# nurturenature/jepsen-tigerbeetle

Measured on AMD Instinct MI355X. Metric: histories/sec, 10k-op/64-proc cas-register histories (time-to-verdict ms in extra), higher is better.
Workload: dtype u64

## Files before the change

### jepsen-tigerbeetle_amd/csrc/batch_run.hip

```cpp
#include "tbc_batch.h"
#include "witness_expand.h"

using namespace tbc;

namespace tbc {

static SearchArgs make_search_args(tbc_batch* B, uint64_t* tab, uint32_t n_work) {
  SearchArgs a{};
  a.hist = B->d_hist.p; a.rec = B->d_rec.p; a.seg = B->d_seg.p; a.ret_slot = B->d_ret_slot.p;
  a.ret_op = B->d_ret_op.p;
  a.frames = B->d_frames.p; a.tab = tab; a.results = B->d_results.p;
  a.witness = B->opts.want_witness ? B->d_witness.p : nullptr;
  a.work = B->d_work.p; a.queue = B->d_queue.p;
  a.table = B->d_table.p; a.n_work = n_work; a.model_kind = B->model.kind;
  a.init_state = B->model.init;
  a.n_classes = B->model.n_classes; a.n_states = B->model.n_states;
  a.max_steps = B->opts.max_steps;
  a.time_limit_ticks = B->opts.time_limit_ms * 100000ull;
  a.dbg = debug_words();
  a.pool_vals = B->d_pool_vals.p;
  a.cfg = B->d_cfg.p;
  a.progress = B->progress; a.progress_dev = B->d_progress.p;
  return a;
}
// ... 352 lines not shown
        restart_budget((ph == 0 && !b->sweep && b->order_restarts_apply()) ? 32ull * b->max_ops : 0ull),
        stall_on(b->lanes != 0 && (b->opts.dominance & TBC_DOM_STALL_HANDOVER) != 0 && !b->count_form && b->mask_words == 1 && !b->opts.want_witness && b->opts.max_steps == 0 && ph == 0 &&
                 (b->model.kind == TBC_MODEL_REGISTER || b->model.kind == TBC_MODEL_CAS_REGISTER) && b->vpad != 0),
        was_handed(b->n_hist, 0), rs_level(b->n_hist, kInf), rs_valid(b->n_hist, 0),
        max_bytes(b->opts.max_visited_bytes ? b->opts.max_visited_bytes : (1ull << 30)) {
    if (B->sweep || B->rsweep) {
      swa.hist = B->d_hist.p; swa.bh = B->d_bh.p; swa.off = B->d_off.p; swa.ncr = B->d_ncr.p; swa.lst = B->d_lst.p;
      swa.crashed = B->d_crashed.p; swa.twn = B->reg_rules() ? B->d_twn.p : nullptr; swa.rdm = B->reg_rules() ? B->d_rdm.p : nullptr;
      swa.slot8 = B->d_slot8.p; swa.cuts = B->d_cuts.p; swa.seg = B->d_sres.p; swa.table = B->d_table.p;
      swa.pool_vals = B->d_pool_vals.p; swa.n_hist = nh; swa.max_segs = B->max_segs; swa.seg_target = B->seg_target;
      swa.cut_open = B->cut_open; swa.n_dom = B->n_dom; swa.vpad = B->vpad ? B->vpad : 1; swa.rules = B->rules;
      swa.model_kind = B->model.kind; swa.init_state = B->model.init;
      swa.n_classes = B->model.n_classes; swa.n_keys = B->model.n_keys;
      swa.shard_rank = 0; swa.shard_world = 1;
    }
  }
};

tbc_status queue_pack(RunState& R) {
  tbc_batch* B = R.B; hipStream_t s = R.s; const uint32_t nh = R.nh; const bool beam = R.beam;
  bool packed = false, counted = false;
  if (nh <= 8) {
    bool fits = true, fits2 = beam;
    for (uint32_t h = 0; h < nh; h++) {
      fits = fits && pack_one_fits(B->model.kind, B->hist[h].n_ops, B->hist[h].n_events, B->hist[h].n_slots);
      fits2 = fits2 && pack_one_counts_fits(B->model.kind, B->hist[h].n_ops, B->hist[h].n_events, B->hist[h].n_slots);
    }
    if (fits2) packed = counted = launch_pack_one_counts(make_pack_args(B), make_pack_open_args(B), s);
    if (!packed && fits) packed = launch_pack_one(make_pack_args(B), s);
  }
  if (!packed && beam) {
    bool fits = true, slots64 = true;
    for (uint32_t h = 0; h < nh && fits; h++) {
      fits = pack_wg_fits(B->model.kind, B->hist[h].n_ops, B->hist[h].n_events, B->hist[h].n_slots);
      slots64 = slots64 && pack_wg64_fits(B->model.kind, B->hist[h].n_ops, B->hist[h].n_events, B->hist[h].n_slots);
    }
    if (fits) packed = counted = launch_pack_wg(make_pack_args(B), make_pack_open_args(B), s, slots64);
  }
  if (!packed) launch_pack(make_pack_args(B), s);
  HIP_TRY(hipGetLastError());
  if (beam) {
    PackOpenArgs po = make_pack_open_args(B);
    if (B->assign_lists) {
      if (!counted) { launch_open_counts(po, s); HIP_TRY(hipGetLastError()); counted = true; }
      tbc_status as = stream_assign_lists(B);
      if (as != TBC_OK) return as;
    }
    launch_pack_open(po, s, counted);
    HIP_TRY(hipGetLastError());
  }
  return TBC_OK;
}

tbc_status first_pass(RunState& R) {
  tbc_batch* B = R.B; hipStream_t s = R.s; const uint32_t nh = R.nh; const bool beam = R.beam; const int phase = R.phase;
  HostBuf<Hist>& hist_back = R.hist_back; HostBuf<BeamHist>& bh_back = R.bh_back;
  TRACE("run: begin");
  HIP_TRY(hipEventRecord(B->ev[0], s));
  if (B->d_progress.p) HIP_TRY(hipMemsetAsync(B->d_progress.p, 0, sizeof(uint32_t), s));
  const bool zero_block = B->borrowed && !guard_on() && !B->d_bitmap.owned && !B->d_off.owned && !B->d_ncr.owned && !B->d_pool_cursor.owned &&
                          (char*)B->d_bitmap.p < (char*)B->d_pool_cursor.p && (size_t)((char*)B->d_pool_cursor.p - (char*)B->d_bitmap.p) < (64u << 20) &&
                          (char*)B->d_off.p > (char*)B->d_bitmap.p && (char*)B->d_off.p < (char*)B->d_pool_cursor.p &&
                          (char*)B->d_ncr.p > (char*)B->d_bitmap.p && (char*)B->d_ncr.p < (char*)B->d_pool_cursor.p;
  const bool fresh = B->inputs_fresh;
  B->inputs_fresh = false;
  if (zero_block) HIP_TRY(hipMemsetAsync(B->d_bitmap.p, 0, (size_t)((char*)B->d_pool_cursor.p - (char*)B->d_bitmap.p) + sizeof(unsigned long long), s));
  else HIP_TRY(hipMemsetAsync(B->d_bitmap.p, 0, B->d_bitmap.bytes(), s));
  const bool use_epoch = beam && B->lanes != 0;
  if (beam) {
    if (use_epoch) B->epoch = B->epoch % 255u + 1u;
    if (!B->sweep && (!use_epoch || B->epoch == 1u)) HIP_TRY(hipMemsetAsync(B->d_btab.p, 0, B->d_btab.bytes(), s));
    if (!B->sweep) HIP_TRY(hipMemsetAsync(B->d_pool.p, 0, B->d_pool.bytes(), s));
    if (!zero_block) {
      HIP_TRY(hipMemsetAsync(B->d_pool_cursor.p, 0, sizeof(unsigned long long), s));
      HIP_TRY(hipMemsetAsync(B->d_off.p, 0, B->d_off.bytes(), s));
      HIP_TRY(hipMemsetAsync(B->d_ncr.p, 0, B->d_ncr.bytes(), s));
    }
    if (!fresh) HIP_TRY(hipMemcpyAsync(B->d_bh.p, B->bh.data(), nh * sizeof(BeamHist), hipMemcpyHostToDevice, s));
  } else {
    HIP_TRY(hipMemsetAsync(B->d_tab.p, 0, B->d_tab.bytes(), s));
  }
  if (!fresh) HIP_TRY(hipMemcpyAsync(B->d_hist.p, B->hist.data(), nh * sizeof(Hist), hipMemcpyHostToDevice, s));
  HIP_TRY(hipEventRecord(B->ev[1], s));
  TRACE("run: memsets queued");
  SYNC_TRACE("memsets");

  if (!B->hist_order.empty()) {
    if (B->d_order.n < nh) { B->d_order.release(); const tbc_status os = B->d_order.alloc(nh); if (os != TBC_OK) return os; }
    HIP_TRY(hipMemcpyAsync(B->d_order.p, B->hist_order.data(), (size_t)nh * 4, hipMemcpyHostToDevice, s));
  }
  tbc_status ps = queue_pack(R);
  if (ps != TBC_OK) return ps;
  TRACE("run: pack launched");
  SYNC_TRACE("pack");
  HIP_TRY(hipEventRecord(B->ev[2], s));

  bool rs_on = B->rsweep && phase == 0 && beam && !B->lanes;
  SweepArgs ra = R.swa;
  if (rs_on) {
    ra.ncr = B->d_zncr.p; ra.crashed = nullptr; ra.reach = B->d_reach.p; ra.reach_hdr = B->d_reach_hdr.p;
    ra.rules = B->rules & (kRuleEager | kRuleTwin);
    HIP_TRY(hipMemsetAsync(B->d_abort.p, 0, B->d_abort.bytes(), s));
    HIP_TRY(hipEventRecord(B->ev2[0], s));
    HIP_TRY(hipStreamWaitEvent(B->stream2, B->ev2[0], 0));
    hist_back.resize(nh);
    if (launch_sweep(ra, B->stream2)) {
      HIP_TRY(hipGetLastError());
      HIP_TRY(hipMemcpyAsync(B->seg_host.data(), B->d_sres.p, B->seg_host.size() * sizeof(SegResult), hipMemcpyDeviceToHost, B->stream2));
      HIP_TRY(hipMemcpyAsync(hist_back.data(), B->d_hist.p, nh * sizeof(Hist), hipMemcpyDeviceToHost, B->stream2));
    } else rs_on = false;
  }

  if (B->sweep) {
    SweepArgs mine = R.swa;
    if (phase == 1 && B->shard_world > 1) {
      mine.shard_rank = B->shard_rank; mine.shard_world = B->shard_world;
      HIP_TRY(hipMemsetAsync(B->d_sres.p, 0, B->d_sres.bytes(), s));
    }
    if (!launch_sweep(mine, s)) { set_error("level sweep launch failed"); return TBC_ERR_HIP; }
  } else if (beam) {
    BeamArgs ba = make_beam_args(B, B->d_btab.p, B->d_stack.p, B->d_dstack.p, nh);
    if (R.first_budget()) ba.max_steps = R.first_budget();
    if (rs_on) ba.abort = B->d_abort.p;
    if (B->lanes) { ba.tab_stride = B->tab_stride(); ba.epoch = use_epoch ? B->epoch : 0u; }
    if (R.stall_on) ba.stall_checks = kStallChecks;
// ... 688 lines not shown
```

### jepsen-tigerbeetle_amd/csrc/batch_stream.hip

```cpp
#include "tbc_batch.h"

using namespace tbc;

namespace tbc {
namespace {

enum : uint32_t { kInBadValue = 1u, kInBadCrashed = 2u };
constexpr uint32_t kMaxInputSlots = 16;

__global__ __launch_bounds__(256) void stream_unpack_kernel(const uint32_t* __restrict__ word, const uint32_t* __restrict__ inv, const uint32_t* __restrict__ ret, uint64_t T,
                                                            uint8_t* __restrict__ of, int32_t* __restrict__ oa, int32_t* __restrict__ ob, int32_t* __restrict__ op,
                                                            uint32_t* __restrict__ oinv, uint32_t* __restrict__ oret, uint32_t vmax, uint32_t allow_crashed, uint32_t* flags) {
  const uint64_t i4 = ((uint64_t)blockIdx.x * blockDim.x + threadIdx.x) * 4ull;
  if (i4 >= T) return;
  uint32_t bad = 0u;
  const auto one = [&](uint32_t w, uint32_t r, uint32_t& f, int32_t& a, int32_t& b, int32_t& p) {
    f = w & 15u;
    const uint32_t a8 = (w >> 4) & 0xFFu, b8 = (w >> 12) & 0xFFu;
    a = a8 == TBC_WIRE_NIL ? TBC_NIL : (int32_t)a8;
    b = b8 == TBC_WIRE_NIL ? TBC_NIL : (int32_t)b8;
    p = (int32_t)(w >> 20);
    if (f <= TBC_F_CAS && ((a8 != TBC_WIRE_NIL && a8 > vmax) || (f == TBC_F_CAS && b8 != TBC_WIRE_NIL && b8 > vmax))) bad |= kInBadValue;
    if (r == TBC_POS_CRASHED && !allow_crashed) bad |= kInBadCrashed;
  };
// ... 75 lines not shown
  HIP_TRY(hipHostMalloc((void**)&B->in_flags_host, 4 * sizeof(uint32_t), hipHostMallocDefault));
  B->in_hist_cap = B->n_hist;
  B->in_ops_cap = ((B->total_ops + B->total_ops / 8 + 1023ull) & ~1023ull) + 1024ull;
  return TBC_OK;
}

size_t slot_bytes(const tbc_batch* B) {
  const size_t a = ((size_t)(B->in_hist_cap + 1) * 8 + 255) & ~(size_t)255, b = ((size_t)B->in_hist_cap * 4 + 255) & ~(size_t)255;
  return a + 2 * b + 3 * (size_t)B->in_ops_cap * 4;
}
void slot_pointers(const tbc_batch* B, char* mem, tbc_batch_input* out) {
  const size_t a = ((size_t)(B->in_hist_cap + 1) * 8 + 255) & ~(size_t)255, b = ((size_t)B->in_hist_cap * 4 + 255) & ~(size_t)255;
  out->n_hist_cap = B->in_hist_cap; out->reserved0 = 0; out->ops_cap = B->in_ops_cap;
  out->op_off = (uint64_t*)mem;
  out->n_events = (uint32_t*)(mem + a);
  out->n_process = (uint32_t*)(mem + a + b);
  out->word = (uint32_t*)(mem + a + 2 * b);
  out->inv_pos = out->word + B->in_ops_cap;
  out->ret_pos = out->inv_pos + B->in_ops_cap;
}

template <typename T>
tbc_status ensure(DevBuf<T>& buf, uint64_t need, bool* grew) {
  if (buf.p && buf.n >= need) return TBC_OK;
  *grew = true;
  return buf.regrow((size_t)(need + need / 16));
}

tbc_status ensure_arenas(tbc_batch* B, const LayoutTotals& t) {
  const uint64_t T = t.total_ops;
  const uint32_t nhc = B->in_hist_cap, MW = B->mask_words;
  bool grew = false, grew_tab = false;
  tbc_status s;
  if ((s = ensure(B->d_f, T, &grew)) || (s = ensure(B->d_a, T, &grew)) || (s = ensure(B->d_b, T, &grew)) || (s = ensure(B->d_proc, T, &grew)) ||
      (s = ensure(B->d_inv, T, &grew)) || (s = ensure(B->d_ret, T, &grew)) || (s = ensure(B->d_ret_slot, T, &grew)) || (s = ensure(B->d_ret_op, T, &grew)) ||
      (s = ensure(B->d_bitmap, t.bm_n, &grew)) || (s = ensure(B->d_wpre, t.bm_n, &grew)) || (s = ensure(B->d_off, t.boff_n, &grew)) || (s = ensure(B->d_ncr, t.boff_n, &grew)) ||
      (s = ensure(B->d_rec, t.rec_n, &grew)) || (s = ensure(B->d_seg, t.seg_n, &grew)) || (s = ensure(B->d_frames, t.frame_n, &grew)) ||
      (s = ensure(B->d_slot8, slot8_bytes(T, nhc), &grew)) || (s = ensure(B->d_stack, t.bstack_n, &grew)))
    return s;
  if (B->opts.want_witness && (s = ensure(B->d_witness, T, &grew))) return s;
  if (B->any_crashed && !B->count_form && (s = ensure(B->d_crashed, T, &grew))) return s;
  if (B->count_form && (s = ensure(B->d_cmem, t.bocc_n, &grew))) return s;
  if (B->lanes && (s = ensure(B->d_rk8, slot8_bytes(T, nhc), &grew))) return s;
  if (B->lanes) { if ((s = ensure(B->d_rdm, T * B->front_words(), &grew))) return s; }
  else if (B->reg_rules() && (s = ensure(B->d_rdm, T * B->vpad * MW, &grew))) return s;
  if (B->lookahead) {
    const bool by_front = MW == 1 && B->vpad <= 32;
    if ((s = ensure(B->d_look, look_words(T, nhc, MW), &grew)) || (!by_front && (s = ensure(B->d_looktmp, T, &grew))) || (s = ensure(B->d_dstack, t.bstack_n, &grew))) return s;
  }
  if ((s = ensure(B->d_btab, t.btab_n * B->tab_stride(), &grew_tab))) return s;
  if (grew_tab) {
    B->epoch = 0;
    const uint64_t words = std::min<uint64_t>(t.btab_n * B->tab_stride() * (B->lanes ? 1u : 3u) / 10, (32ull << 30) / 8);
    if (words > B->d_pool.n && (s = B->d_pool.regrow(words))) return s;
  }
  (void)grew;
  return TBC_OK;
}

tbc_status plan_count_input(tbc_batch* B, const tbc_batch_input& in, uint32_t* planned, uint32_t nh, tbc_pending_input& P, std::vector<uint32_t>& n_slots) {
  P.count_hist.assign(nh, CountHist{});
  n_slots.assign(nh, 1u);
  std::vector<uint64_t> lists(nh, 0);
  const bool cas_model = B->model.kind == TBC_MODEL_CAS_REGISTER;
  const unsigned hw = std::max(1u, std::thread::hardware_concurrency());
  const unsigned nt = in.op_off[nh] > (1ull << 20) ? std::min(16u, hw) : 1u;
  std::vector<int> bad(nt, -1);
  const auto work = [&](unsigned t) {
    std::vector<uint8_t> f; std::vector<int32_t> a, b, proc, slot; std::vector<uint32_t> rets, pre; std::vector<int32_t> slot_of; std::vector<uint8_t> used;
    for (uint32_t h = (uint32_t)((uint64_t)nh * t / nt); h < (uint32_t)((uint64_t)nh * (t + 1) / nt); h++) {
      const uint64_t o0 = in.op_off[h], n = in.op_off[h + 1] - o0;
      f.resize(n); a.resize(n); b.resize(n); proc.resize(n); slot.assign(n + 1, 0);
      for (uint64_t i = 0; i < n; i++) {
        const uint32_t w = in.word[o0 + i], a8 = (w >> 4) & 0xFFu, b8 = (w >> 12) & 0xFFu;
        f[i] = (uint8_t)(w & 15u); a[i] = a8 == TBC_WIRE_NIL ? TBC_NIL : (int32_t)a8; b[i] = b8 == TBC_WIRE_NIL ? TBC_NIL : (int32_t)b8; proc[i] = (int32_t)(w >> 20);
      }
      tbc_ops c{};
      c.n = (uint32_t)n; c.f = f.data(); c.a = a.data(); c.b = b.data(); c.process = proc.data(); c.inv_pos = in.inv_pos + o0; c.ret_pos = in.ret_pos + o0;
      if (!build_count_form(c, 0, n, in.n_process[h], cas_model, slot.data(), P.count_hist[h], rets, slot_of, used)) { if (bad[t] < 0) bad[t] = (int)h; continue; }
      n_slots[h] = std::max(1u, P.count_hist[h].n_slots);
      for (uint64_t i = 0; i < n; i++) planned[o0 + i] = (in.word[o0 + i] & 0xFFFFFu) | ((uint32_t)slot[i] << 20);
      c.process = slot.data();
      lists[h] = open_list_entries(c, 0, n, in.n_events[h], n_slots[h], pre, false);
    }
  };
  if (nt == 1) work(0);
  else {
    std::vector<std::thread> th;
    for (unsigned t = 0; t < nt; t++) th.emplace_back(work, t);
    for (auto& x : th) x.join();
  }
  for (int h : bad) if (h >= 0) {
    set_error("history %d of the input: its crashed calls do not fit the count form (more than 128 bits of counts, or a process number out of range): destroy and create", h);
    return TBC_ERR_UNSUPPORTED;
  }
  size_t words = 0;
  for (uint32_t h = 0; h < nh; h++) { words += P.count_hist[h].words.size(); P.lst_total += std::max<uint64_t>(1, lists[h]); }
  P.cmem.clear(); P.cmem.reserve(words);
  for (uint32_t h = 0; h < nh; h++) P.cmem.insert(P.cmem.end(), P.count_hist[h].words.begin(), P.count_hist[h].words.end());
  return TBC_OK;
}

}

void stream_release(tbc_batch* B) {
  for (auto& sl : B->in_slots) {
    if (sl.copied) { (void)hipEventSynchronize(sl.copied); (void)hipEventDestroy(sl.copied); }
// ... 263 lines not shown
```

### jepsen-tigerbeetle_amd/csrc/open_walk_impl.h

```cpp
#pragma once
#include "wave_env.h"
#include "tbc_internal.h"

namespace tbc {
namespace walk {

constexpr uint32_t kCandCap = 136;
constexpr uint32_t kCandWords = 8;
constexpr uint32_t kAuxWords = 80;
WV_HD constexpr uint32_t walk_lds_words() { return kCandCap * kCandWords + kAuxWords; }

constexpr uint32_t kCList = 1u;
constexpr uint32_t kCTwin = 2u;
constexpr uint32_t kCRow = 4u;
constexpr uint32_t kCLook = 8u;

WV_DEV void or_slot(uint32_t& lo, uint32_t& hi, bool cond, uint32_t slot) {
  if (slot < 32u) lo = wv::opaque(lo | (cond ? (1u << slot) : 0u));
  else hi = wv::opaque(hi | (cond ? (1u << (slot - 32u)) : 0u));
}
WV_DEV uint32_t effect_key(uint32_t f, int32_t a, int32_t b) {
  return (f & 3u) | (((uint32_t)a & 0x7FFFu) << 2) | ((f == TBC_F_CAS ? ((uint32_t)b & 0x7FFFu) : 0u) << 17);
}
static_assert(kMaxRuleValue < 0x7FFF && TBC_F_READ < 3 && TBC_F_WRITE < 3 && TBC_F_CAS < 3, "effect_key packs f and two rule values into a word, and no key has all bits set");
static_assert(kLookNone <= 0xFFu, "the produced value shares a word with the flags");

WV_DEV uint32_t rank_code(uint32_t slot, uint32_t f, int32_t a, uint32_t vpad) {
  const uint32_t k8 = f == TBC_F_READ ? (rdm_index(a, vpad) & 0xFFu) : 0xFFu;
  return (slot & 63u) | ((k8 == 0xFFu ? 7u : (k8 & 7u)) << 6);
}

template <int Q>
WV_DEV void store_entries(const wv::u32x16& r, uint64_t* row, uint32_t n) {
  WV_UNROLL
  for (int v = 0; v < 8; v++) if ((uint32_t)(8 * Q + v) < n) row[8 * Q + v] = (uint64_t)r[2 * v] | ((uint64_t)r[2 * v + 1] << 32);
}

template <int VCAP>
WV_DEV void walk_wave(const PackOpenArgs& A, uint32_t wid, uint32_t* lds, uint32_t lane) {
  const uint32_t cph = A.chunks_per_hist;
  const uint32_t hr = wid / cph, c = wid - hr * cph, h = A.h0 + hr;
  if (h >= A.n_hist) return;
  const Hist* H = &A.hist[h];
  const BeamHist* B = &A.bh[h];
  const uint32_t R = H->n_ret;
  const uint32_t F_lo = c * 64u;
  if (H->status != 0 || B->status != 0 || F_lo >= R) return;
  const uint32_t F_hi = F_lo + 64u < R ? F_lo + 64u : R;
  const uint32_t W = H->n_slots;
  const Rec* rec = A.rec + H->rec_off;
  const uint32_t* seg = A.seg + H->seg_off;
  const uint32_t* off = A.off + B->off_off;
  OpRec* lst = A.lst + B->lst_off;
  uint64_t* twn = A.twn ? A.twn + B->lst_off : nullptr;
  const uint32_t V = A.vpad;
  const uint32_t FW = A.front_words ? A.front_words : V;
  const bool compact = A.front_compact != 0u;
  uint64_t* rdm = (A.rdm && (V || compact)) ? A.rdm + H->op_off * FW : nullptr;
  const bool want_tw = twn != nullptr;
  uint64_t* look = A.look ? A.look + look_off(H->op_off, h, 1u) : nullptr;
  uint32_t* cand = lds;
  uint32_t* aux = lds + kCandCap * kCandWords;
// ... 11 lines not shown
    uint32_t i = lo;
    for (;;) {
      const uint32_t i1 = i + 1u < tail ? i + 1u : tail, i2 = i + 2u < tail ? i + 2u : tail, i3 = i + 3u < tail ? i + 3u : tail;
      const uint32_t v0 = rec[i < tail ? i : tail].inv_rank, v1 = rec[i1].inv_rank, v2 = rec[i2].inv_rank, v3 = rec[i3].inv_rank;
      if (v0 >= F_hi) break;
      i++;
      if (v1 >= F_hi) break;
      i++;
      if (v2 >= F_hi) break;
      i++;
      if (v3 >= F_hi) break;
      i++;
    }
    k = i - lo;
  }
  uint32_t incl = k;
  for (uint32_t d = 1; d < 64u; d <<= 1) {
    aux[lane] = incl;
    wv::barrier();
    const uint32_t add = lane >= d ? aux[lane - d] : 0u;
    wv::barrier();
    incl += add;
  }
  const uint32_t base = incl - k;
  const uint32_t NC_all = wv::readlane(incl, 63u);
  const uint32_t NC = NC_all < kCandCap ? NC_all : kCandCap;
  for (uint32_t j = 0; j < k; j++) {
    const Rec r = rec[lo + j];
    if (base + j < kCandCap) {
      const bool live = (r.cls & 2u) != 0u, isread = (r.cls & 16u) != 0u, wc = (r.cls & 8u) != 0u;
      const bool in_chunk = r.ret_rank >= F_lo;
      const bool listed = live && in_chunk && !(A.branch_lists && isread);
      const uint32_t vi = rdm_index(r.a, V);
      uint32_t fl = (lane << 12) | (r.prod << 24);
      if (listed) fl |= kCList;
      if (listed && wc && want_tw) fl |= kCTwin;
      if (live && in_chunk && isread && rdm && V && (vi != 0u || r.a == TBC_NIL)) fl |= kCRow | (vi << 4);
      if (look && (r.cls & 6u) && r.prod != kLookNone) fl |= kCLook;
      uint32_t* e = cand + (base + j) * kCandWords;
      e[0] = r.inv_rank; e[1] = r.ret_rank; e[2] = r.opidx; e[3] = r.f | (lane << 8);
      e[4] = (uint32_t)r.a; e[5] = (uint32_t)r.b; e[6] = fl;
      e[7] = (live && wc && in_chunk) ? effect_key(r.f, r.a, r.b) : 0xFFFFFFFFu;
    }
  }
  wv::barrier();

  const uint32_t list_order = A.order_of ? A.order_of[h] : A.list_order;
  const bool by_ret = list_order != 0u;
  const uint32_t wr_last = list_order == 2u ? 0x40000000u : list_order >= 16u ? 2u * (list_order - 16u) + 1u : 0u;
  const uint32_t rk_mul = list_order >= 16u ? 2u : 1u;
  uint16_t* const perm = reinterpret_cast<uint16_t*>(aux);
  if (by_ret) {
    uint32_t my[3], place[3] = {0u, 0u, 0u};
    WV_UNROLL
    for (int s = 0; s < 3; s++) {
      const uint32_t idx = lane + 64u * (uint32_t)s;
      const uint32_t* e = cand + (idx < NC ? idx : 0u) * kCandWords;
      const uint32_t rt = e[1];
      my[s] = idx >= NC ? 0xFFFFFFFFu : rt == kInf ? (0xFFFFFF00u | idx) : rt * rk_mul + ((e[3] & 0xFFu) == TBC_F_WRITE ? wr_last : 0u);
    }
    const uint32_t n0 = NC < 64u ? NC : 64u, n1 = NC <= 64u ? 0u : (NC < 128u ? NC - 64u : 64u), n2 = NC <= 128u ? 0u : NC - 128u;
    if (NC <= 64u) {
      for (uint32_t j = 0; j < n0; j++) place[0] += wv::readlane(my[0], j) < my[0] ? 1u : 0u;
    } else if (NC <= 128u) {
      for (uint32_t j = 0; j < n0; j++) { const uint32_t kj = wv::readlane(my[0], j); place[0] += kj < my[0] ? 1u : 0u; place[1] += kj < my[1] ? 1u : 0u; }
      for (uint32_t j = 0; j < n1; j++) { const uint32_t kj = wv::readlane(my[1], j); place[0] += kj < my[0] ? 1u : 0u; place[1] += kj < my[1] ? 1u : 0u; }
    } else {
      WV_UNROLL
      for (int s2 = 0; s2 < 3; s2++) {
        const uint32_t cnt = s2 == 0 ? n0 : s2 == 1 ? n1 : n2;
        for (uint32_t j = 0; j < cnt; j++) {
          const uint32_t kj = wv::readlane(my[s2], j);
          place[0] += kj < my[0] ? 1u : 0u; place[1] += kj < my[1] ? 1u : 0u; place[2] += kj < my[2] ? 1u : 0u;
        }
      }
    }
    WV_UNROLL
    for (int s = 0; s < 3; s++) {
      const uint32_t idx = lane + 64u * (uint32_t)s;
      if (idx < NC) perm[place[s]] = (uint16_t)idx;
    }
    wv::barrier();
  }

  uint32_t c_key[3] = {0xFFFFFFFFu, 0xFFFFFFFFu, 0xFFFFFFFFu}, c_ret[3] = {0u, 0u, 0u};
  if (want_tw) {
    WV_UNROLL
    for (int s = 0; s < 3; s++) {
      const uint32_t idx = lane + 64u * (uint32_t)s;
      const uint32_t* e = cand + (idx < NC ? idx : 0u) * kCandWords;
      c_key[s] = idx < NC ? e[7] : 0xFFFFFFFFu;
      c_ret[s] = e[1];
    }
  }

  const uint32_t F = F_lo + lane;
  const bool active = F < F_hi;
  const uint32_t Fc = active ? F : F_hi - 1u;
  const uint32_t pos0 = off[Fc];
  uint32_t pos = pos0;
  const uint32_t px = A.ret_slot[H->ret_off + Fc];
  uint32_t need = kLookNone, xprod = kLookNone, di = 0, x = 0, xf = kFNone;
  int32_t xa = 0;
  if (look || compact) {
    x = A.ret_op[H->ret_off + Fc];
    xf = A.f[H->op_off + x];
    xa = A.a[H->op_off + x];
  }
  if (look) {
    const int32_t xb = A.b[H->op_off + x];
    const uint32_t xinv = A.scratch[H->frame_off + x];
    need = look_need(xf, xa); xprod = look_prod(xf, xa, xb);
    di = F - xinv < 255u ? F - xinv : 255u;
  }
  wv::u32x16 r0, r1, r2, r3;
// ... 92 lines not shown
```

### jepsen-tigerbeetle_amd/csrc/pack_one_impl.h

```cpp
#pragma once
#include "tbc_internal.h"
#include "wave_env_wg.h"

namespace tbc {
namespace packone {

template <uint32_t NW_, uint32_t MAXEV_, uint32_t MAXW_, uint32_t MAXR_, uint32_t HBITS_ = 16>
struct Geo {
  static constexpr uint32_t kNW = NW_, kT = 64 * NW_, kMaxEvents = MAXEV_, kMaxW = MAXW_, kMaxR = MAXR_, kHBits = HBITS_, kHPer = 32 / HBITS_;
  static_assert((HBITS_ == 8 || HBITS_ == 16) && MAXW_ < (1u << HBITS_), "a histogram entry counts up to one call per slot");
  static constexpr bool kCounts = MAXR_ != 0;
  static constexpr uint32_t kBmWords = MAXEV_ / 32 + 32;
  static constexpr uint32_t kOffBm = 0, kOffPre = kBmWords, kOffCnt = 2 * kBmWords, kOffSeg = kOffCnt + NW_ * MAXW_,
                            kOffTot = kOffSeg + MAXW_ + 8, kOffFlag = kOffTot + 2 * NW_, kOffHist = kOffFlag + 8,
                            kHistWords = kCounts ? MAXR_ / kHPer + 4 : 0, kOffRdb = kOffHist + kHistWords,
                            kRdbWords = kCounts ? MAXR_ / 32 + 2 : 0, kLdsWords = kOffRdb + kRdbWords;
  WV_HD static constexpr uint32_t lds_words() { return kLdsWords; }
  WV_HD static bool fits(uint32_t model_kind, uint32_t n_ops, uint32_t n_events, uint32_t n_slots) {
    const bool model_ok = model_kind == TBC_MODEL_REGISTER || model_kind == TBC_MODEL_CAS_REGISTER || model_kind == TBC_MODEL_MUTEX ||
                          model_kind == TBC_MODEL_TABLE;
    return model_ok && n_events <= kMaxEvents && n_slots <= kMaxW && (!kCounts || n_ops <= kMaxR);
  }
};
using OneGeo = Geo<16, 131072, kMaxSlots, 0>;
using OneCountsGeo = Geo<16, 131072, kMaxSlots, 16384>;
using BatchGeo = Geo<4, 32768, 256, 8192>;
using Batch64Geo = Geo<4, 32768, 64, 8192, 8>;

constexpr uint32_t kNW = OneGeo::kNW;
WV_HD constexpr uint32_t lds_words() { return OneGeo::lds_words(); }
WV_HD inline bool fits(uint32_t model_kind, uint32_t n_ops, uint32_t n_events, uint32_t n_slots) { return OneGeo::fits(model_kind, n_ops, n_events, n_slots); }

WV_DEV bool op_ok(uint32_t kind, uint32_t f, int32_t a, uint32_t n_classes) {
  return kind == TBC_MODEL_REGISTER ? (f == TBC_F_READ || f == TBC_F_WRITE)
       : kind == TBC_MODEL_CAS_REGISTER ? (f == TBC_F_READ || f == TBC_F_WRITE || f == TBC_F_CAS)
       : kind == TBC_MODEL_MUTEX ? (f == TBC_F_ACQUIRE || f == TBC_F_RELEASE)
       : (kind == TBC_MODEL_TABLE && f == TBC_F_CLASS && (uint32_t)a < n_classes);
}

#define TBC_PACK_ONE_SCAN(out_, total_, x_, flip_)                                                                        \
  do {                                                                                                                   \
    uint32_t y_ = (x_);                                                                                                  \
    y_ += wv::row_shr0<1>(y_); y_ += wv::row_shr0<2>(y_); y_ += wv::row_shr0<4>(y_); y_ += wv::row_shr0<8>(y_);          \
    const uint32_t t0_ = wv::readlane(y_, 15u), t1_ = wv::readlane(y_, 31u), t2_ = wv::readlane(y_, 47u), t3_ = wv::readlane(y_, 63u); \
    const uint32_t row_ = lane >> 4;                                                                                     \
    y_ += (row_ > 0u ? t0_ : 0u) + (row_ > 1u ? t1_ : 0u) + (row_ > 2u ? t2_ : 0u);                                      \
    uint32_t* tt_ = tot + ((flip_) ? G::kNW : 0u);                                                                          \
    if (lane == 0u) tt_[wave] = t0_ + t1_ + t2_ + t3_;                                                                   \
    wv::wg_barrier();                                                                                                    \
    uint32_t base_ = 0u, all_ = 0u;                                                                                      \
    for (uint32_t w_ = 0; w_ < G::kNW; w_++) { const uint32_t v_ = wv::lds_ld32(&tt_[w_]); base_ += w_ < wave ? v_ : 0u; all_ += v_; } \
    (out_) = base_ + y_ - (x_);                                                                                          \
    (total_) = all_;                                                                                                     \
  } while (0)

template <class G>
WV_DEV void history(const PackArgs& A, const PackOpenArgs& O, uint32_t* lds) {
  constexpr uint32_t kT = G::kT;
  static_assert(G::kMaxW <= G::kT, "one thread per process slot in the list-start scan");
  const uint32_t tid = wv::wg_thread(), lane = tid & 63u, wave = tid >> 6;
  const uint32_t h = A.h0 + wv::wg_index();
  if (h >= A.n_hist) return;
  Hist* H = &A.hist[h];
  const uint32_t n = H->n_ops, W = H->n_slots, E = H->n_events;
// ... 82 lines not shown
    return;
  }

  uint32_t R;
  {
    const uint32_t per = (nw + kT - 1u) / kT;
    const uint32_t lo = tid * per < nw ? tid * per : nw, hi = lo + per < nw ? lo + per : nw;
    uint32_t sum = 0u;
    for (uint32_t w = lo; w < hi; w++) sum += (uint32_t)__builtin_popcount(bm[w]);
    uint32_t run;
    TBC_PACK_ONE_SCAN(run, R, sum, 0);
    for (uint32_t w = lo; w < hi; w++) { pre[w] = run; run += (uint32_t)__builtin_popcount(bm[w]); }
  }
  TBC_PROF_PHASE(2);
  if (R != n_done) {
    if (tid == 0u) { H->n_ret = 0u; H->status = (uint32_t)TBC_ERR_BAD_HISTORY; }
    no_lists();
    return;
  }

  {
    uint32_t mine = 0u;
    if (tid < W) {
      uint32_t run = 0u;
      for (uint32_t k = 0; k < G::kNW; k++) { const uint32_t c = cnt[k * W + tid]; cnt[k * W + tid] = run; run += c; }
      mine = run + 2u;
    }
    uint32_t start, total;
    TBC_PACK_ONE_SCAN(start, total, mine, 1);
    if (tid < W) { seg[tid] = start; A.seg[H->seg_off + tid] = start; }
    if (tid == 0u) { seg[W] = total; A.seg[H->seg_off + W] = total; }
  }
  wv::wg_barrier();
  TBC_PROF_PHASE(3);

  {
    const uint32_t c0 = wave * cpw, c1 = c0 + cpw < chunks ? c0 + cpw : chunks;
    uint32_t* mycnt = cnt + wave * W;
    uint32_t i = c0 * 64u + lane;
    bool in = c0 < c1 && i < n;
    uint32_t n_iv = in ? inv[i] : 0u, n_rt = in ? ret[i] : TBC_POS_CRASHED, n_f = in ? (uint32_t)f[i] : 0u;
    int32_t n_p = in ? proc[i] : 0, n_a = in ? a[i] : 0, n_b = in ? b[i] : 0;
    uint32_t crashed_cands = 0u;
    for (uint32_t c = c0; c < c1; c++) {
      const uint32_t iv = n_iv, rt = n_rt, ff = n_f; const int32_t pp = n_p, aa = n_a, bb = n_b;
      const bool here = in;
      const uint32_t me = i;
      i += 64u;
      in = c + 1u < c1 && i < n;
      n_iv = in ? inv[i] : 0u; n_rt = in ? ret[i] : TBC_POS_CRASHED; n_f = in ? (uint32_t)f[i] : 0u;
      n_p = in ? proc[i] : 0; n_a = in ? a[i] : 0; n_b = in ? b[i] : 0;
      const bool live = here && rt != TBC_POS_CRASHED;
      const uint32_t p = (here && !(cf && rt == TBC_POS_CRASHED)) ? (uint32_t)pp : 0xFFFFFFFFu;
      uint32_t before = 0u;
      for (uint32_t l = 0; l < 64u; l++) {
        const uint32_t pl = wv::readlane(p, l);
        before += (pl == p && l < lane) ? 1u : 0u;
      }
      const bool slotted = p != 0xFFFFFFFFu;
      uint32_t dst = kInf;
      if (slotted) dst = seg[p] + 1u + mycnt[p] + before;
      wv::barrier();
      if (slotted) wv::lds_add32(&mycnt[p], 1u);
      wv::barrier();
      if (here) {
        const uint32_t ir = pre[iv >> 5] + (uint32_t)__builtin_popcount(bm[iv >> 5] & ((1u << (iv & 31u)) - 1u));
        uint32_t rr = kInf;
        if (live) {
          rr = pre[rt >> 5] + (uint32_t)__builtin_popcount(bm[rt >> 5] & ((1u << (rt & 31u)) - 1u));
          A.ret_slot[H->ret_off + rr] = (uint32_t)pp;
          A.ret_op[H->ret_off + rr] = me;
        }
        sc_inv[me] = ir; sc_ret[me] = rr; sc_dst[me] = dst;
        if (slotted) {
          Rec r;
          r.inv_rank = ir; r.ret_rank = rr; r.opidx = me; r.f = ff; r.a = aa; r.b = bb;
          r.cls = rec_cls(ff, aa, rr == kInf); r.prod = look_prod(ff, aa, bb);
          rec[dst] = r;
        }
        if constexpr (G::kCounts) {
          const bool isread = ff == TBC_F_READ;
          if (live) {
            slot8[rr] = (uint8_t)pp;
            if (rk8) rk8[rr] = isread ? (uint8_t)rdm_index(aa, O.vpad) : (uint8_t)0xFF;
            if (branch && isread) wv::lds_or32(&rdb[rr >> 5], 1u << (rr & 31u));
            else wv::lds_add32_wg(&hist[ir / G::kHPer], 1u << (G::kHBits * (ir % G::kHPer)));
          } else if (!cf && !(isread && aa == TBC_NIL)) {
            crashed_cands++;
            if (ir < R) atomicAdd(&ncr[ir], 1u);
          }
        }
      }
    }
    if (G::kCounts && crashed_cands) wv::lds_add32_wg(&flag[2], crashed_cands);
  }
  TBC_PROF_PHASE(4);
  for (uint32_t p = tid; p < W; p += kT) {
    Rec hd; hd.inv_rank = 0; hd.ret_rank = 0; hd.opidx = kInf; hd.f = kFNone; hd.a = 0; hd.b = 0; hd.cls = 0; hd.prod = kLookNone;
    Rec tl = hd; tl.inv_rank = kInf; tl.ret_rank = kInf;
    rec[seg[p]] = hd;
    rec[seg[p + 1u] - 1u] = tl;
  }
  wv::wg_fence();
  wv::wg_barrier();
  TBC_PROF_PHASE(5);

  {
    const uint32_t c0 = wave * cpw, c1 = c0 + cpw < chunks ? c0 + cpw : chunks;
    uint32_t err = 0u;
    for (uint32_t c = c0; c < c1; c += 4u) {
      uint32_t d[4], iv[4], pr[4], pf[4];
      WV_UNROLL
// ... 86 lines not shown
```

### jepsen-tigerbeetle_amd/csrc/tbc_batch.h

```cpp
#pragma once
#include <hip/hip_runtime.h>
#include <algorithm>
#include <atomic>
#include <chrono>
#include <cstdio>
#include <cstdlib>
#include <cstring>
#include <deque>
#include <mutex>
#include <new>
#include <thread>
#include <vector>
#include "tbc_internal.h"

namespace tbc {

#define HIP_TRY(expr)                                                             \
  do {                                                                            \
    hipError_t e_ = (expr);                                                       \
    if (e_ != hipSuccess) {                                                       \
      ::tbc::set_error("%s failed: %s (%s:%d)", #expr, hipGetErrorString(e_), __FILE__, __LINE__); \
      return e_ == hipErrorOutOfMemory ? TBC_ERR_OOM : TBC_ERR_HIP;               \
    }                                                                             \
  } while (0)

inline uint32_t ceil_log2(uint64_t x) {
  uint32_t l = 0;
  while ((1ull << l) < x) l++;
  return l;
}

uint64_t now_ns();
bool device_is_gfx950(int dev);
uint32_t* debug_words();
#define SYNC_TRACE(msg) do { if (std::getenv("TBC_SYNC_EACH")) { hipError_t e__ = hipStreamSynchronize(s); std::fprintf(stderr, "[tbc sync] %s -> %s\n", msg, hipGetErrorString(e__)); std::fflush(stderr); } } while (0)
#define TRACE(msg) do { if (std::getenv("TBC_DEBUG")) { std::fprintf(stderr, "[tbc %9.3f ms] %s\n", (double)(::tbc::now_ns() % 100000000000ull) / 1e6, msg); std::fflush(stderr); } } while (0)

struct Ctx {
  int device = 0;
  char* slab = nullptr;
  size_t cap = 0, used = 0, wanted = 0;
  char* pin = nullptr;
  size_t pin_cap = 0, pin_used = 0, pin_wanted = 0;
  hipStream_t stream = nullptr;
  hipEvent_t ev[6] = {};
  hipStream_t stream2 = nullptr;
  hipEvent_t ev2[2] = {};
};
extern thread_local Ctx* t_ctx;
Ctx* ctx_acquire(int device);
void ctx_release(Ctx* c);
struct CtxSuspend {
  Ctx* const saved;
  CtxSuspend() : saved(t_ctx) { t_ctx = nullptr; }
  ~CtxSuspend() { t_ctx = saved; }
};

bool guard_on();
constexpr size_t kGuardBytes = 256;
extern thread_local const void* t_guard_owner;
extern thread_local size_t t_guard_nth;
void guard_add(const void* arena_end);
void guard_remove(const void* arena_end);
size_t guard_check(const char* when, const void* owner);

template <typename T>
// ... 130 lines not shown
  std::vector<uint32_t> hist_order;
  tbc::DevBuf<uint32_t> d_order;
  tbc::DevBuf<uint32_t> d_park;
  uint32_t last_raced = 0;
  uint32_t* progress = nullptr;
  tbc::DevBuf<uint32_t> d_progress;
  mutable std::atomic<uint32_t> progress_seen{0};
  std::atomic<uint64_t> run_t0{0};
  std::atomic<uint32_t> running{0};
  bool order_restarts_apply() const {
    return width > 1 && !lanes && !count_form && list_order_applies() && opts.list_order == TBC_ORDER_DEFAULT && opts.max_steps == 0 &&
           !(opts.dominance & TBC_DOM_NO_ORDER_RESTARTS);
  }
  std::vector<tbc::BeamHist> bh;
  tbc::DevBuf<tbc::BeamHist> d_bh;
  tbc::DevBuf<uint32_t> d_off, d_ncr, d_stack;
  tbc::DevBuf<tbc::OpRec> d_lst, d_crashed;
  tbc::DevBuf<uint8_t> d_slot8;
  tbc::DevBuf<uint8_t> d_rk8;
  bool lookahead = false;
  tbc::DevBuf<uint64_t> d_look;
  tbc::DevBuf<uint32_t> d_dstack;
  tbc::DevBuf<uint32_t> d_looktmp;
  bool sweep = false;
  uint32_t max_segs = 1, seg_target = 0, cut_open = 0, n_dom = 1;
  tbc::DevBuf<uint32_t> d_cuts, d_seglist;
  tbc::DevBuf<tbc::SegResult> d_sres;
  tbc::HostBuf<tbc::SegResult> seg_host;
  bool rsweep = false;
  tbc::DevBuf<uint32_t> d_zncr, d_reach, d_reach_hdr, d_abort;
  hipStream_t stream2 = nullptr;
  hipEvent_t ev2[2] = {};
  uint32_t* abort_one = nullptr;
  uint32_t last_segments = 0, last_fallback = 0;
  uint32_t shard_rank = 0, shard_world = 1;
  bool partial_done = false;
  tbc::HostBuf<tbc::Hist> hist_back_m;
  tbc::HostBuf<tbc::BeamHist> bh_back_m;
  tbc::HostBuf<char> upload_stage;
  bool inputs_fresh = false;
  uint32_t rules = 0;
  uint32_t vpad = 0;
  tbc::DevBuf<uint64_t> d_twn, d_rdm;
  tbc::DevBuf<uint64_t> d_occ, d_btab, d_pool;
  bool count_form = false;
  tbc::DevBuf<uint64_t> d_cmem;
  std::vector<tbc::CountHist> count_hist;
  uint32_t reg_rules() const { return rules & (tbc::kRuleEager | tbc::kRuleTwin); }
  uint32_t epoch = 0;
  bool any_crashed = true;
  uint32_t tab_stride() const { return entry_words() - ((lanes && !opts.want_witness) ? 1u : 0u); }
  uint32_t entry_words() const { return mask_words + 2u + (count_form ? tbc::kCountWords : 0u); }
  tbc::DevBuf<unsigned long long> d_pool_cursor;
  std::vector<tbc::DevResult> res_host;
  std::vector<uint32_t> witness_host;
  uint64_t timing_ns[4] = {0, 0, 0, 0};
  hipEvent_t ev_turn = nullptr;
  uint64_t turn_wait_ns = 0;
  tbc_counters sum{};
  uint64_t device_bytes = 0;
  void count_device_bytes();

  struct InputSlot { char* mem = nullptr; size_t bytes = 0; hipEvent_t copied = nullptr; bool busy = false; uint32_t* planned = nullptr; };
  std::vector<InputSlot> in_slots;
  uint32_t in_hist_cap = 0;
  uint64_t in_ops_cap = 0;
  tbc::DevBuf<uint32_t> d_stage[2];
  hipStream_t stream_copy = nullptr;
  hipEvent_t ev_stage[2] = {};
  hipEvent_t ev_unpacked[2] = {};
  bool stage_used[2] = {false, false};
  uint64_t in_seq = 0;
  std::deque<tbc_pending_input> pending;
  tbc::DevBuf<uint32_t> d_in_flags;
  uint32_t* in_flags_host = nullptr;
  bool assign_lists = false;
  tbc::DevBuf<uint32_t> d_list_over;
  uint64_t in_bytes_copied = 0, in_copy_ns = 0;
  hipEvent_t ev_copy[2][2] = {};
  tbc::LayoutTotals cap;
  bool lists_headroom = false;
  bool inputs_stale = false;
  uint64_t inputs_consumed = 0;
  uint32_t lists_regrown = 0, reload_slot = 0;

  bool borrowed = false;
  ~tbc_batch();
};

namespace tbc {

struct ColumnScan { bool nonneg = true, any_crashed = false, any_crashed_effect = false; int32_t vmax = -1; };
ColumnScan scan_columns(const tbc_ops& c, uint64_t T);
tbc_status layout_histories(tbc_batch* B, uint32_t nh, const uint64_t* op_off, const uint32_t* n_events, const uint32_t* n_slots, const int32_t* aux,
                            const uint32_t* list_caps, bool lists_on_device, std::vector<Hist>& hist, std::vector<BeamHist>& bh, LayoutTotals& tot,
                            const std::vector<CountHist>* count_hist = nullptr);
bool build_count_form(const tbc_ops& c, uint64_t o0, uint64_t n, uint32_t n_process, bool cas_model, int32_t* slot_col, CountHist& out,
                      std::vector<uint32_t>& rets, std::vector<int32_t>& slot_of, std::vector<uint8_t>& used);
uint64_t open_list_entries(const tbc_ops& c, uint64_t op_off, uint64_t n, uint32_t n_events, uint32_t n_slots, std::vector<uint32_t>& pre, bool branch_lists);
tbc_status batch_create_impl(const tbc_batch_desc* desc, const tbc_model* model, const tbc_opts* opts, tbc_batch* B);

PackArgs make_pack_args(tbc_batch* B);
PackOpenArgs make_pack_open_args(tbc_batch* B);
tbc_status batch_run_impl(tbc_batch* B, tbc_result* results, int phase = 0);

tbc_status stream_consume(tbc_batch* B, bool* consumed);
// ... 6 lines not shown
```

Before: 393,300.

## Zero only written pool range, bitmap-rank candidate ordering, ballot-based slot ranking

Three separate changes. First, the pool memset is replaced, after the first run, by a kernel that zeroes only the prefix up to the cursor left by the previous pass. This cuts memory traffic, but the pool must stay clean between runs. Second, the open walk's O(NC) readlane rank loop gets a bitmap-plus-prefix-scan rank in LDS when the candidate return keys fall inside a 1024-bit window. Third, the pack kernel's 64-iteration readlane loop that counts earlier lanes with the same proc is replaced by per-bit ballots.

```diff
diff --git a/jepsen-tigerbeetle_amd/csrc/batch_run.hip b/jepsen-tigerbeetle_amd/csrc/batch_run.hip
--- a/jepsen-tigerbeetle_amd/csrc/batch_run.hip
+++ b/jepsen-tigerbeetle_amd/csrc/batch_run.hip
@@ -428,6 +428,16 @@
   return TBC_OK;
 }
 
+constexpr uint32_t kPoolZeroBlocks = 1024, kPoolZeroThreads = 256;
+__global__ __launch_bounds__(kPoolZeroThreads) void pool_zero_written_kernel(uint64_t* __restrict__ pool, const unsigned long long* __restrict__ cursor, uint64_t pool_words) {
+  const uint64_t n = pool_written(*cursor, pool_words);
+  const uint64_t stride = (uint64_t)gridDim.x * kPoolZeroThreads * 2u;
+  for (uint64_t i = ((uint64_t)blockIdx.x * kPoolZeroThreads + threadIdx.x) * 2u; i < n; i += stride) {
+    if (i + 1u < n) *reinterpret_cast<ulonglong2*>(pool + i) = make_ulonglong2(0ull, 0ull);
+    else pool[i] = 0ull;
+  }
+}
+
 tbc_status first_pass(RunState& R) {
   tbc_batch* B = R.B; hipStream_t s = R.s; const uint32_t nh = R.nh; const bool beam = R.beam; const int phase = R.phase;
   HostBuf<Hist>& hist_back = R.hist_back; HostBuf<BeamHist>& bh_back = R.bh_back;
@@ -446,7 +456,14 @@
   if (beam) {
     if (use_epoch) B->epoch = B->epoch % 255u + 1u;
     if (!B->sweep && (!use_epoch || B->epoch == 1u)) HIP_TRY(hipMemsetAsync(B->d_btab.p, 0, B->d_btab.bytes(), s));
-    if (!B->sweep) HIP_TRY(hipMemsetAsync(B->d_pool.p, 0, B->d_pool.bytes(), s));
+    if (!B->sweep) {
+      const bool whole = pool_zero_whole(B->pool_state, use_epoch, B->epoch);
+      if (whole || zero_block) HIP_TRY(hipMemsetAsync(B->d_pool.p, 0, B->d_pool.bytes(), s));
+      else {
+        hipLaunchKernelGGL(pool_zero_written_kernel, dim3(kPoolZeroBlocks), dim3(kPoolZeroThreads), 0, s, B->d_pool.p, B->d_pool_cursor.p, (uint64_t)B->d_pool.n);
+        HIP_TRY(hipGetLastError());
+      }
+    }
     if (!zero_block) {
       HIP_TRY(hipMemsetAsync(B->d_pool_cursor.p, 0, sizeof(unsigned long long), s));
       HIP_TRY(hipMemsetAsync(B->d_off.p, 0, B->d_off.bytes(), s));
diff --git a/jepsen-tigerbeetle_amd/csrc/batch_stream.hip b/jepsen-tigerbeetle_amd/csrc/batch_stream.hip
--- a/jepsen-tigerbeetle_amd/csrc/batch_stream.hip
+++ b/jepsen-tigerbeetle_amd/csrc/batch_stream.hip
@@ -151,7 +151,7 @@
   if (grew_tab) {
     B->epoch = 0;
     const uint64_t words = std::min<uint64_t>(t.btab_n * B->tab_stride() * (B->lanes ? 1u : 3u) / 10, (32ull << 30) / 8);
-    if (words > B->d_pool.n && (s = B->d_pool.regrow(words))) return s;
+    if (words > B->d_pool.n) { B->pool_state.replaced(); if ((s = B->d_pool.regrow(words))) return s; }
   }
   (void)grew;
   return TBC_OK;
diff --git a/jepsen-tigerbeetle_amd/csrc/open_walk_impl.h b/jepsen-tigerbeetle_amd/csrc/open_walk_impl.h
--- a/jepsen-tigerbeetle_amd/csrc/open_walk_impl.h
+++ b/jepsen-tigerbeetle_amd/csrc/open_walk_impl.h
@@ -8,6 +8,8 @@
 constexpr uint32_t kCandCap = 136;
 constexpr uint32_t kCandWords = 8;
 constexpr uint32_t kAuxWords = 80;
+constexpr uint32_t kKeyWords = 32, kKeyBits = 32 * kKeyWords;
+static_assert(2 * kKeyWords <= kAuxWords && kKeyWords == 32, "the map and its prefix fit the scratch; two rows of 16 lanes scan it");
 WV_HD constexpr uint32_t walk_lds_words() { return kCandCap * kCandWords + kAuxWords; }
 
 constexpr uint32_t kCList = 1u;
@@ -125,15 +127,51 @@
   uint16_t* const perm = reinterpret_cast<uint16_t*>(aux);
   if (by_ret) {
     uint32_t my[3], place[3] = {0u, 0u, 0u};
+    uint32_t d[3];
+    const uint32_t wr_ofs = list_order == 2u ? kKeyBits / 2u : wr_last, lim_other = list_order == 2u ? kKeyBits / 2u : kKeyBits;
+    bool outside = false;
     WV_UNROLL
     for (int s = 0; s < 3; s++) {
       const uint32_t idx = lane + 64u * (uint32_t)s;
       const uint32_t* e = cand + (idx < NC ? idx : 0u) * kCandWords;
       const uint32_t rt = e[1];
-      my[s] = idx >= NC ? 0xFFFFFFFFu : rt == kInf ? (0xFFFFFF00u | idx) : rt * rk_mul + ((e[3] & 0xFFu) == TBC_F_WRITE ? wr_last : 0u);
+      const bool wr = (e[3] & 0xFFu) == TBC_F_WRITE;
+      my[s] = idx >= NC ? 0xFFFFFFFFu : rt == kInf ? (0xFFFFFF00u | idx) : rt * rk_mul + (wr ? wr_last : 0u);
+      const bool live = idx < NC && rt != kInf;
+      const uint32_t x = rt - ret_from;
+      const bool inside = x < kKeyBits && x * rk_mul + (wr ? wr_ofs : 0u) < (wr ? kKeyBits : lim_other);
+      d[s] = (live && inside) ? x * rk_mul + (wr ? wr_ofs : 0u) : kInf;
+      outside = outside || (live && !inside);
     }
     const uint32_t n0 = NC < 64u ? NC : 64u, n1 = NC <= 64u ? 0u : (NC < 128u ? NC - 64u : 64u), n2 = NC <= 128u ? 0u : NC - 128u;
-    if (NC <= 64u) {
+    if (wr_ofs < kKeyBits && wv::ballot(outside) == 0ull) {
+      if (lane < kKeyWords) aux[lane] = 0u;
+      wv::barrier();
+      WV_UNROLL
+      for (int s = 0; s < 3; s++) if (d[s] != kInf) wv::lds_add32(&aux[d[s] >> 5], 1u << (d[s] & 31u));
+      wv::barrier();
+      const uint32_t wc = lane < kKeyWords ? (uint32_t)__builtin_popcount(aux[lane]) : 0u;
+      uint32_t y = wc;
+      y += wv::row_shr0<1>(y); y += wv::row_shr0<2>(y); y += wv::row_shr0<4>(y); y += wv::row_shr0<8>(y);
+      const uint32_t row0 = wv::readlane(y, 15u);
+      y += lane >= 16u ? row0 : 0u;
+      const uint32_t n_live = wv::readlane(y, kKeyWords - 1u);
+      if (lane < kKeyWords) aux[kKeyWords + lane] = y - wc;
+      const uint64_t below = (1ull << lane) - 1ull;
+      uint32_t cr_before = n_live;
+      WV_UNROLL
+      for (int s = 0; s < 3; s++) {
+        const uint32_t idx = lane + 64u * (uint32_t)s;
+        const uint64_t cr = wv::ballot(idx < NC && d[s] == kInf);
+        if (d[s] == kInf) place[s] = cr_before + (uint32_t)__builtin_popcountll(cr & below);
+        cr_before += (uint32_t)__builtin_popcountll(cr);
+      }
+      wv::barrier();
+      WV_UNROLL
+      for (int s = 0; s < 3; s++)
+        if (d[s] != kInf) place[s] = aux[kKeyWords + (d[s] >> 5)] + (uint32_t)__builtin_popcount(aux[d[s] >> 5] & ((1u << (d[s] & 31u)) - 1u));
+      wv::barrier();
+    } else if (NC <= 64u) {
       for (uint32_t j = 0; j < n0; j++) place[0] += wv::readlane(my[0], j) < my[0] ? 1u : 0u;
     } else if (NC <= 128u) {
       for (uint32_t j = 0; j < n0; j++) { const uint32_t kj = wv::readlane(my[0], j); place[0] += kj < my[0] ? 1u : 0u; place[1] += kj < my[1] ? 1u : 0u; }
diff --git a/jepsen-tigerbeetle_amd/csrc/pack_one_impl.h b/jepsen-tigerbeetle_amd/csrc/pack_one_impl.h
--- a/jepsen-tigerbeetle_amd/csrc/pack_one_impl.h
+++ b/jepsen-tigerbeetle_amd/csrc/pack_one_impl.h
@@ -4,12 +4,15 @@
 
 namespace tbc {
 namespace packone {
+
+WV_HD constexpr uint32_t slot_bits(uint32_t max_w) { uint32_t b = 0; while (b < 32u && (1ull << b) < max_w) b++; return b; }
 
 template <uint32_t NW_, uint32_t MAXEV_, uint32_t MAXW_, uint32_t MAXR_, uint32_t HBITS_ = 16>
 struct Geo {
   static constexpr uint32_t kNW = NW_, kT = 64 * NW_, kMaxEvents = MAXEV_, kMaxW = MAXW_, kMaxR = MAXR_, kHBits = HBITS_, kHPer = 32 / HBITS_;
   static_assert((HBITS_ == 8 || HBITS_ == 16) && MAXW_ < (1u << HBITS_), "a histogram entry counts up to one call per slot");
   static constexpr bool kCounts = MAXR_ != 0;
+  static constexpr uint32_t kSlotBits = slot_bits(MAXW_);
   static constexpr uint32_t kBmWords = MAXEV_ / 32 + 32;
   static constexpr uint32_t kOffBm = 0, kOffPre = kBmWords, kOffCnt = 2 * kBmWords, kOffSeg = kOffCnt + NW_ * MAXW_,
                             kOffTot = kOffSeg + MAXW_ + 8, kOffFlag = kOffTot + 2 * NW_, kOffHist = kOffFlag + 8,
@@ -198,12 +201,15 @@
       n_p = in ? proc[i] : 0; n_a = in ? a[i] : 0; n_b = in ? b[i] : 0;
       const bool live = here && rt != TBC_POS_CRASHED;
       const uint32_t p = (here && !(cf && rt == TBC_POS_CRASHED)) ? (uint32_t)pp : 0xFFFFFFFFu;
-      uint32_t before = 0u;
-      for (uint32_t l = 0; l < 64u; l++) {
-        const uint32_t pl = wv::readlane(p, l);
-        before += (pl == p && l < lane) ? 1u : 0u;
-      }
       const bool slotted = p != 0xFFFFFFFFu;
+      uint64_t same = wv::ballot(slotted);
+      WV_UNROLL
+      for (uint32_t bit = 0; bit < G::kSlotBits; bit++) {
+        const bool set = ((p >> bit) & 1u) != 0u;
+        const uint64_t m = wv::ballot(slotted && set);
+        same &= set ? m : ~m;
+      }
+      const uint32_t before = (uint32_t)__builtin_popcountll(same & ((1ull << lane) - 1ull));
       uint32_t dst = kInf;
       if (slotted) dst = seg[p] + 1u + mycnt[p] + before;
       wv::barrier();
diff --git a/jepsen-tigerbeetle_amd/csrc/pool_plan.h b/jepsen-tigerbeetle_amd/csrc/pool_plan.h
--- /dev/null
+++ b/jepsen-tigerbeetle_amd/csrc/pool_plan.h
@@ -0,0 +1,25 @@
+#pragma once
+#include <cstdint>
+
+#if defined(__HIPCC__)
+#define TBC_POOL_HD __host__ __device__
+#else
+#define TBC_POOL_HD
+#endif
+
+namespace tbc {
+
+struct PoolState {
+  bool clean = false;
+  void replaced() { clean = false; }
+};
+
+TBC_POOL_HD inline uint64_t pool_written(uint64_t cursor, uint64_t pool_words) { return cursor < pool_words ? cursor : pool_words; }
+
+inline bool pool_zero_whole(PoolState& st, bool use_epoch, uint32_t epoch) {
+  const bool whole = !st.clean || (use_epoch && epoch == 1u);
+  st.clean = true;
+  return whole;
+}
+
+}
diff --git a/jepsen-tigerbeetle_amd/csrc/tbc_batch.h b/jepsen-tigerbeetle_amd/csrc/tbc_batch.h
--- a/jepsen-tigerbeetle_amd/csrc/tbc_batch.h
+++ b/jepsen-tigerbeetle_amd/csrc/tbc_batch.h
@@ -12,6 +12,7 @@
 #include <thread>
 #include <vector>
 #include "tbc_internal.h"
+#include "pool_plan.h"
 
 namespace tbc {
 
@@ -248,6 +249,7 @@
   uint32_t tab_stride() const { return entry_words() - ((lanes && !opts.want_witness) ? 1u : 0u); }
   uint32_t entry_words() const { return mask_words + 2u + (count_form ? tbc::kCountWords : 0u); }
   tbc::DevBuf<unsigned long long> d_pool_cursor;
+  tbc::PoolState pool_state;
   std::vector<tbc::DevResult> res_host;
   std::vector<uint32_t> witness_host;
   uint64_t timing_ns[4] = {0, 0, 0, 0};
```

New measurement: 404,200, median of 6. 2.8% higher.
